# swacisko/ALGA

Measured on AMD Instinct MI355X. Metric: overlap_edges_per_sec, higher is better.
Workload: dtype u32; 1 GPU; cfg4_50M_150bp: 50000000 x 150 bp reads, genome 250000000, seed 11, err 0.00 -> 90621096 nodes (both strands, duplicates removed), min_overlap 82, rsoemo 116; generated on the device (alga_amd.workload.device_build) in 1.0 s; nodes=90621096, edges=92350115

## Files before the change

alga_amd/csrc/engine.hip:

```cpp
#include <hip/hip_runtime.h>

#include <algorithm>
#include <chrono>
#include <cstdio>
#include <cstdlib>
#include <cstring>
#include <new>
#include <string>
#include <thread>
#include <vector>

#include "engine_internal.h"
#include "prefsuf_shard.h"

using namespace alga;

namespace {

using Prepared = AlgaPrepared;

int prepare(alga_engine *e, const alga_nodes *nodes, const alga_prefsuf_params *p, hipStream_t s, Prepared &out) {
    if (!nodes || !p) return alga_fail(e, ALGA_ERR_INVALID_ARGUMENT, "nodes/params must not be NULL");
    if (nodes->n < 0) return alga_fail(e, ALGA_ERR_INVALID_ARGUMENT, "negative node count");
    if (nodes->n > 0 && (!nodes->words || !nodes->len)) return alga_fail(e, ALGA_ERR_INVALID_ARGUMENT, "words/len must not be NULL");
// ... 203 lines not shown
                HIP_TRY(e, hipEventRecord(e->ev[EV_DIR], s));
            }
            HIP_TRY(e, launch_cluster_gather(nd, cc, pp.cluster_eq, (const uint32_t *) e->cl_keys[1].p, (const uint32_t *) e->cl_vals[1].p, (const uint32_t *) e->cl_meta.p,
                                             pp.uniform_len, e->cl_store.p, (pile && e->opt_pile_skip_gather) ? (const unsigned long long *) e->cl_pile_cnt.p : nullptr, s));
            HIP_TRY(e, hipEventRecord(e->ev[EV_GATHER], s));
            if (pile) {
                if (e->pile_epoch >= 511u) {
                    HIP_TRY(e, hipMemsetAsync(e->cl_pile_tab.p, 0, e->cl_pile_tab.cap, s));
                    e->pile_epoch = 0;
                }
                e->pile_epoch++;
                const bool from_consensus = e->opt_pile_runs != 0;
                launch_pile_build(nd, cfg, cc, pp.uniform_len, (const uint32_t *) e->cl_keys[1].p, (const uint32_t *) e->cl_vals[1].p, e->cl_dir.p, e->cl_pile_rec.p, e->cl_pile_rec2.p, e->cl_pile_tab.p,
                                  e->pile_epoch, e->cl_pile_succ.p, e->cl_runs.p, pp.uniform_len - cfg.Lmin + 1, (const unsigned long long *) e->cl_pile_cnt.p,
                                  from_consensus ? (uint32_t *) e->cl_pile_own.p : nullptr, (from_consensus && e->opt_pile_runs_list) ? e->cl_pile_list.p : nullptr, s,
                                  e->opt_pile_dir >= 1, cnt + CNT_TOTAL + 1, e->pile_tab_index);
                if ((rc = alga_check_launch(e, "k_pile_build"))) return rc;
                if (keys_only) {
                    launch_pile_own_ids((const uint32_t *) e->cl_pile_own.p, (const uint32_t *) e->cl_vals[1].p, (uint64_t) nd.n, (int32_t *) e->cl_defer.p, (uint32_t) nd.n,
                                        (unsigned long long *) e->cl_pile_cnt.p, s);
                    launch_cluster_runs_list(nd, cfg, cc, (const int32_t *) e->cl_defer.p, (const unsigned long long *) e->cl_pile_cnt.p + 3, (uint32_t) nd.n, (uint32_t) e->n_cu * 16u,
                                             e->cl_runs.p, (uint8_t *) e->cl_nruns.p, s);
                    launch_cluster_keys(nd, cfg, cc, 0, nd.n, (uint32_t *) e->cl_keys[0].p, (uint32_t *) e->cl_vals[0].p, (uint32_t *) e->cl_meta.p, e->cl_runs.p,
                                        (uint8_t *) e->cl_nruns.p, s, true, (const unsigned long long *) e->cl_pile_cnt.p);
                    if ((rc = alga_check_launch(e, "k_node_runs (own lists)"))) return rc;
                }
                if (e->opt_pile_check && from_consensus)
                    launch_pile_check(e->cl_pile_succ.p, (uint64_t) nd.n, cc.n_buckets, e->cl_pile_tab.p, e->cl_pile_rec2.p, e->pile_epoch, e->cl_runs.p, nd.n, pp.uniform_len - cfg.Lmin + 1,
                                      (unsigned long long *) e->cl_pile_cnt.p, s);
                e->pile_n = nd.n; e->pile_words = (const void *) nd.words;
                e->pile_keys_only = keys_only; e->pile_kept_pure = false;
// ... 32 lines not shown
                if ((rc = alga_ensure(e, e->cl_defer, (size_t) (n_src + 64) * sizeof(int32_t)))) return rc;
                const uint32_t slot_stride = e->opt_stream_slots >= 4 ? (uint32_t) (n_src + 1) : 0u;
                if ((rc = alga_ensure(e, e->loc_second, (size_t) (slot_stride ? LOCAL_SLOTS_MAX - 1 : 1) * (n_src + 1) * sizeof(unsigned long long)))) return rc;
                e->loc_second_used = true;
                e->loc_slot_stride = slot_stride;
                const bool by_key = e->opt_cluster_order != 0 && src_begin == 0 && src_end == nd.n;
                const bool piled = pile && e->pile_n == nd.n && e->pile_words == (const void *) nd.words;
                if (piled) {
                    if (!all_sources) {
                        if ((rc = alga_ensure(e, e->cl_pile_side_r, (size_t) (n_src + 64) * 16))) return rc;
                        if ((rc = alga_ensure(e, e->cl_pile_cursor, 64))) return rc;
                    }
                    launch_pile_probe(nd, cfg, cc, pp.uniform_len, e->cl_pile_tab.p, e->pile_epoch, e->cl_pile_rec.p, e->cl_pile_rec2.p, e->cl_pile_succ.p,
                                      e->cl_runs.p, cnt, (uint32_t *) e->outdeg.p, (unsigned long long *) e->loc_first.p, (unsigned long long *) e->loc_second.p,
                                      (int32_t *) e->cl_defer.p, (uint32_t) n_src, (const unsigned long long *) e->cl_pile_cnt.p, e->n_cu, s, src_begin, src_end,
                                      e->cl_pile_side_r.p, (unsigned long long *) e->cl_pile_cursor.p, e->opt_pile_probe_lean != 0);
                    if ((rc = alga_check_launch(e, "k_pile_probe"))) return rc;
                    if (keys_only)
                        launch_cluster_runs_list(nd, cfg, cc, (const int32_t *) e->cl_defer.p, cnt + CNT_DEFERRED, (uint32_t) std::min<uint64_t>(n_src + 64, 0xFFFFFFFFull),
                                                 (uint32_t) e->n_cu * 16u, e->cl_runs.p, (uint8_t *) e->cl_nruns.p, s);
                }
                launch_probe_stream(nd, cfg, cc, pp.cluster_eq, e->cl_store.p, e->cl_dir.p, e->cl_runs.p, (const uint8_t *) e->cl_nruns.p,
                                    src_begin, src_end, by_key, cnt, e->n_cu, (uint32_t *) e->outdeg.p, (unsigned long long *) e->loc_first.p,
                                    (unsigned long long *) e->loc_second.p, (int32_t *) e->cl_defer.p, (uint32_t) n_src,
                                    piled ? (const unsigned long long *) e->cl_pile_cnt.p : nullptr, s, slot_stride);
                if ((rc = alga_check_launch(e, "k_probe_stream"))) return rc;
                if (piled) {
                    if ((rc = alga_ensure(e, e->cl_defer2, (size_t) (n_src + 64) * sizeof(int32_t)))) return rc;
                    pure_streamed = launch_probe_stream_list(nd, cfg, cc, pp.cluster_eq, e->cl_store.p, e->cl_dir.p, e->cl_runs.p, (const uint8_t *) e->cl_nruns.p, (int32_t *) e->cl_defer.p,
                                             (uint32_t) n_src, cnt, e->n_cu, (uint32_t *) e->outdeg.p, (unsigned long long *) e->loc_first.p,
                                             (unsigned long long *) e->loc_second.p, (int32_t *) e->cl_defer2.p, (const unsigned long long *) e->cl_pile_cnt.p, s, slot_stride, src_begin,
// ... 325 lines not shown
    } else if (!strcmp(name, "pile")) {
        e->opt_pile = (value == 2 || value == 3) ? (int) value : (value != 0);
    } else if (!strcmp(name, "pile_runs")) {
        e->opt_pile_runs = value != 0;
    } else if (!strcmp(name, "pile_runs_list")) {
        e->opt_pile_runs_list = value != 0;
    } else if (!strcmp(name, "pile_dir")) {
        if (value < 0 || value > 2) return alga_fail(e, ALGA_ERR_INVALID_ARGUMENT, "option pile_dir: 0 directory records, 1 k_pile_build from the keys, 2 ... and no directory for a pure pile build");
        e->opt_pile_dir = (int) value;
    } else if (!strcmp(name, "pile_deg_fold")) {
        e->opt_pile_deg_fold = value != 0;
    } else if (!strcmp(name, "emit_fused")) {
        e->opt_emit_fused = value != 0;
    } else if (!strcmp(name, "pile_probe_lean")) {
        e->opt_pile_probe_lean = value != 0;
    } else if (!strcmp(name, "pile_stream_by_id")) {
        e->opt_pile_stream_by_id = value != 0;
    } else if (!strcmp(name, "pile_check")) {
        e->opt_pile_check = value != 0;
    } else if (!strcmp(name, "pile_skip_gather")) {
        e->opt_pile_skip_gather = value != 0;
    } else if (!strcmp(name, "cluster_order")) {
        e->opt_cluster_order = value != 0;
    } else if (!strcmp(name, "local_big_max")) {
        e->big_limit = value < 0 ? -1 : (int) std::min<int64_t>(value, 1 << 20);
    } else if (!strcmp(name, "shard_bucket_max")) {
        e->opt_shard_dmax = (int) std::max<int64_t>(1, std::min<int64_t>(value, 4096));
    } else if (!strcmp(name, "rsort_variant")) {
        if (value < 0 || value > 1) return alga_fail(e, ALGA_ERR_INVALID_ARGUMENT, "option rsort_variant: 0 tiles of 8192 pairs, 1 tiles of 16384 pairs");
        rsort_set_variant((int) value);
// ... 737 lines not shown
```

alga_amd/csrc/engine_internal.h:

```cpp
#pragma once
#include <hip/hip_runtime.h>

#include <cstdio>
#include <algorithm>
#include <string>
#include <vector>
#include <unordered_map>

#include "../../include/alga_amd.h"
#include "prefsuf_common.h"
#include "prefsuf_kernels.h"
#include "pkb_kernels.h"

struct DevBuf {
    void  *p = nullptr;
    size_t cap = 0;
};

enum { EV_START = 0, EV_SEED, EV_PROBE, EV_GROUP, EV_REDUCE, EV_EMIT, EV_PAIRS, EV_KEYS, EV_SORT, EV_GATHER, EV_DIR, EV_SAMPLE, EV_COUNT };
constexpr int ALGA_STAGE_THREADS = 8;

struct alga_engine {
    std::vector<DevBuf *> owned;
    int         device = -1;
// ... 26 lines not shown
    bool   store_timed = false;
    bool   pile_keys_only = false, pile_kept_pure = false;
    int    opt_pile_range = 1;
    int    opt_pile_skip_gather = 1;
    int    opt_pile = 1;
    int    opt_pile_runs = 1;
    int    opt_pile_runs_list = 1;
    DevBuf cl_pile_list;
    int    opt_pile_deg_fold = 1;
    int    opt_emit_fused = 1;
    int    opt_pile_dir = 2;
    bool   dir_late = false;
    bool   pile_tab_index = false;
    int    opt_pile_stream_by_id = 0;
    int    opt_pile_probe_lean = 1;
    bool   pile_deg_pending = false;
    int    opt_pile_check = 0;
    bool   expect_pairwise = false;
    DevBuf cl_pile_side_r, cl_pile_cursor;
    DevBuf cl_pile_own;
    int    opt_pkb_legacy = 0;
    int    opt_own_sort = 1;
    int    opt_test_presort_oom = 0;
    int    opt_test_pile_oom = 0;
    bool   pile_timed = false;
    DevBuf cl_pile_succ;
    DevBuf cl_pile_rec2;
    DevBuf cl_pile_rec, cl_pile_cnt, cl_pile_tab;
    uint32_t pile_epoch = 0;
    int32_t pile_n = -1; const void *pile_words = nullptr;
// ... 228 lines not shown
```

alga_amd/csrc/prefsuf_kernels.h:

```cpp
#pragma once
#include <hip/hip_runtime.h>
#include <stddef.h>
#include <stdint.h>
#include "prefsuf_common.h"

namespace alga {

struct alga_edge_dev { int32_t src, dst, offset; };

void launch_restride(const uint32_t *in, int stride_in, uint32_t *out, int stride_out, uint64_t n, hipStream_t s);
void launch_widen_len(const void *in, int elem_bytes , int32_t *out, uint64_t n, hipStream_t s);
void launch_compact_edges(const alga_edge_dev *edges, int32_t n, uint64_t n_edges, uint8_t *deg, uint32_t *dst, uint8_t *off, unsigned long long *bad, hipStream_t s);
void launch_expand_twins(const uint32_t *in, int stride_in, const int32_t *len , uint32_t *out, int stride_out, uint64_t n_pairs, hipStream_t s);
void launch_node_stats(const NodesDev &nd, unsigned long long *counters, int *max_len , hipStream_t s);

uint32_t seed_buckets_for(uint64_t live_nodes, int fill_x10);
uint32_t seed_filter_bits_for(uint64_t live_nodes);
void launch_seed_build(const NodesDev &nd, const PrefSufCfg &cfg, unsigned long long *table, uint32_t n_buckets, uint32_t *filter,
                       uint32_t filter_bits, hipStream_t s);

struct ProbeBig { int32_t *list; uint32_t list_cap; uint32_t count; void *items; uint32_t item_cap; };
int    local_item_capacity();
int    local_big_limit();
size_t probe_big_bytes(int n_cu, uint32_t count, int local, uint32_t item_cap);
// ... 43 lines not shown
void       launch_pile_deg(int32_t n, unsigned long long *first, uint32_t *deg, const unsigned long long *pile_cnt, hipStream_t s);
bool       pile_plan(const PrefSufCfg &cfg, const ClusterCfg &cc, int eq, int uniform_len, bool masks);
size_t     pile_record_bytes(uint64_t n);
size_t     pile_table_bytes(uint32_t n_buckets);
void       launch_pile_sample(const NodesDev &nd, const ClusterCfg &cc, int uniform_len, const uint32_t *skeys , const uint32_t *sids , const void *dir,
                              unsigned long long *pile_cnt , int no_sample, hipStream_t s,
                              bool from_keys = false );
constexpr int PILE_CNT_WORDS = 6;
size_t     pile_own_mask_bytes(uint64_t n);
size_t     pile_list_bytes(uint64_t n);
void       launch_pile_build(const NodesDev &nd, const PrefSufCfg &cfg, const ClusterCfg &cc, int uniform_len, const uint32_t *skeys, const uint32_t *sids, const void *dir, void *rec,
                             void *rec2 , void *tab, uint32_t epoch, void *side, const void *runs, int nwin, const unsigned long long *pile_cnt,
                             uint32_t *own_mask ,
                             void *plist , hipStream_t s,
                             bool from_keys = false , unsigned long long *bad_flag = nullptr,
                             bool full_record = false );
void       launch_pile_own_ids(const uint32_t *own_mask, const uint32_t *sids, uint64_t n_entries, int32_t *list, uint32_t cap, unsigned long long *pile_cnt, hipStream_t s);
void       launch_pile_check(const void *side, uint64_t n_entries, uint32_t n_buckets, const void *tab, const void *rec2, uint32_t epoch, const void *runs, int n_nodes, int nwin,
                             unsigned long long *pile_cnt, hipStream_t s);
bool       launch_probe_stream_list(const NodesDev &nd, const PrefSufCfg &cfg, const ClusterCfg &cc, int eq, const void *store, const void *dir, const void *runs, const uint8_t *nruns,
                                    int32_t *src_list, uint32_t list_cap, unsigned long long *counters, int n_cu, uint32_t *deg, unsigned long long *first,
                                    unsigned long long *second, int32_t *defer2, const unsigned long long *pile_cnt, hipStream_t s, uint32_t slot_stride = 0,
                                    int32_t src_base = 0 ,
                                    const uint32_t *skeys = nullptr, const uint32_t *sids = nullptr, int uniform_len = 0, bool by_id = false,
                                    const void *tab = nullptr , uint32_t epoch = 0);
void       launch_pile_probe(const NodesDev &nd, const PrefSufCfg &cfg, const ClusterCfg &cc, int uniform_len, const void *tab, uint32_t epoch, const void *rec, const void *rec2, const void *side,
                             const void *runs, unsigned long long *counters, uint32_t *deg, unsigned long long *first, unsigned long long *second, int32_t *defer_list,
                             uint32_t defer_cap, const unsigned long long *pile_cnt, int n_cu, hipStream_t s, int32_t src_begin, int32_t src_end,
                             void *side_range , unsigned long long *cursor ,
                             bool lean = true );

size_t     rsort_u32_pairs_temp_bytes(uint64_t n);
void       rsort_set_variant(int v);
hipError_t rsort_u32_pairs(void *temp, size_t temp_bytes, const uint32_t *keys_in, uint32_t *keys_out, const uint32_t *vals_in, uint32_t *vals_out, uint64_t n,
                           int begin_bit, hipStream_t s);
size_t     sort_u32_pairs_temp_bytes(uint64_t n);
hipError_t sort_u32_pairs(void *temp, size_t temp_bytes, const uint32_t *keys_in, uint32_t *keys_out, const uint32_t *vals_in, uint32_t *vals_out,
                          uint64_t n, int begin_bit , hipStream_t s, bool own_sort = true );
size_t     rsort_u64_pairs_temp_bytes(uint64_t n);
hipError_t rsort_u64_pairs(void *temp, size_t temp_bytes, const unsigned long long *keys_in, unsigned long long *keys_out, const unsigned long long *vals_in,
                           unsigned long long *vals_out, uint64_t n, int bits, hipStream_t s);
hipError_t rsort_u32_u64(void *temp, size_t temp_bytes, const uint32_t *keys_in, uint32_t *keys_out, const unsigned long long *vals_in, unsigned long long *vals_out,
                         uint64_t n, int begin_bit, int end_bit, hipStream_t s);
size_t     sort_u64_pairs_temp_bytes(uint64_t n, int bits);
hipError_t sort_u64_pairs(void *temp, size_t temp_bytes, const unsigned long long *keys_in, unsigned long long *keys_out,
// ... 42 lines not shown
```

alga_amd/csrc/prefsuf_pile.hip:

```cpp
#include <hip/hip_runtime.h>
#include <algorithm>
#include "prefsuf_common.h"
#include "prefsuf_kernels.h"
#include "prefsuf_device.h"
#include "prefsuf_cluster_device.h"

namespace alga {

constexpr int PB_TILE = 192, PB_HALO = 64, PB_THREADS = PB_TILE + PB_HALO;
constexpr int PILE_SW = 13;
constexpr int PILE_MAXSUB = 4;
constexpr int PILE_EQ = 3;

__device__ __forceinline__ bool pile_declines(const unsigned long long *pile_cnt) { return pile_cnt_declines(pile_cnt); }

__device__ __forceinline__ uint32_t pile_who(uint32_t group, uint32_t w, uint32_t n_buckets, uint64_t n_entries) {
    return group == 0u ? min(w, n_buckets) : (uint32_t) min((uint64_t) w, n_entries) | 0x80000000u;
}

__device__ __forceinline__ void load_row9(const NodesDev &nd, uint32_t id, uint32_t (&row)[9]) {
    const uint32_t *rp = nd.words + (size_t) id * nd.stride;
    if ((nd.stride & 3) == 0 && nd.stride >= 12 && ((uintptr_t) nd.words & 15u) == 0) {
        const uint4 v0 = reinterpret_cast<const uint4 *>(rp)[0], v1 = reinterpret_cast<const uint4 *>(rp)[1];
        row[0] = v0.x; row[1] = v0.y; row[2] = v0.z; row[3] = v0.w; row[4] = v1.x; row[5] = v1.y; row[6] = v1.z; row[7] = v1.w;
// ... 328 lines not shown
                    last_key = k1[r]; last_pos = kpos; c1_last = c1;
                    n++;
                }
            }
        }
    }
    ok = ok && n >= 1 && n <= PILE_RUNS;
    pile_list_store(line, l4.x, ok, n, ok_, kc_, c1_last);
}

constexpr int PR_TILE = 3072;
constexpr int PR_TKW = 21;
constexpr int PR_RCAP = 14;
constexpr int PR_SEGS = 32;

template <int RS, int RW>
__device__ __forceinline__ void pile_consensus_one(uint32_t who, bool in, uint32_t *row, uint32_t (*stk)[TK_ROWS], uint16_t (*rbuf)[TK_ROWS], int t, const uint4 *__restrict__ side,
                                                   uint64_t n_entries, uint4 *__restrict__ tab, const uint4 *__restrict__ rec, uint4 *__restrict__ rec2, const ClusterCfg &cc, int U,
                                                   int Lmin, uint32_t *__restrict__ own_mask) {
    const int fs = cc.idx_shift - CL_MBITS;
    const int step = max(16, min(64, cc.w) & ~15);
    const bool further = (who >> 31) != 0u;
    const uint32_t slot = who & 0x7FFFFFFFu;
    uint4 *line = tab + (size_t) (further ? 0u : who) * 8;
    const uint4 *src = further ? rec + (size_t) slot * 4 : (const uint4 *) line;
    uint32_t S[PILE_SW + 1];
    unsigned long long rm = 0ull;
    {
        const uint4 l0 = src[0], l1 = src[1], l2 = src[2], l3 = src[3];
        S[0] = l0.x; S[1] = l0.y; S[2] = l0.z; S[3] = l0.w; S[4] = l1.x; S[5] = l1.y; S[6] = l1.z; S[7] = l1.w;
        S[8] = l2.x; S[9] = l2.y; S[10] = l2.z; S[11] = l2.w; S[12] = l3.x; S[13] = 0u;
        rm = !in ? 0ull : (further ? (((unsigned long long) l3.w << 32) | l3.z) : (((unsigned long long) l3.z << 32) | l3.y));
    }
    const bool act = in && rm != 0ull;
    const int m_min = act ? __clzll((long long) rm) : 0, m_max = act ? 63 - __builtin_ctzll(rm) : 0;
    const int len_v = U + m_max - m_min;
    const int nwin = len_v - Lmin + 1;
    {
        const int ob = 2 * (64 - m_max), w0 = ob >> 5, sh = ob & 31;
        uint32_t m1 = 0u - (uint32_t) (w0 & 1), m2 = 0u - (uint32_t) ((w0 >> 1) & 1), m4 = 0u - (uint32_t) ((w0 >> 2) & 1);
        asm volatile("" : "+v"(m1), "+v"(m2), "+v"(m4));
        uint32_t y1[PILE_SW + 1], y2[PILE_SW + 1], y[PILE_SW + 1];
#pragma unroll
        for (int k = 0; k <= PILE_SW; k++) y1[k] = ((k + 1 <= PILE_SW ? S[k + 1] : 0u) & m1) | (S[k] & ~m1);
// ... 31 lines not shown
        }
    }
    ok = ok && n >= 1 && n <= PILE_RUNS;
    if (in && further) {
        uint4 *l2 = rec2 + (size_t) slot * 4 - 4;
        pile_list_store(l2, 0u, ok, n, key_, kc_, (uint32_t) (nwin - m_max + 64));
        if (!ok) {
            const uint64_t jb = slot >= 3u ? (uint64_t) slot - 3u : 0ull;
            for (uint64_t j2 = jb; j2 < jb + 64u + 3u && j2 < n_entries; j2++) {
                const uint4 s2 = side[j2];
                if ((s2.z >> 31) && ((s2.z >> 16) & 3u) != 0u && s2.w == slot) atomicOr(&own_mask[j2 >> 5], 1u << (j2 & 31u));
            }
        }
    } else if (in) {
        uint32_t *lw = reinterpret_cast<uint32_t *>(line);
        pile_list_store(line, lw[16], ok, n, key_, kc_, (uint32_t) (nwin - m_max + 64));
        if (!ok) {
            lw[16] = lw[16] & 255u;
            const uint32_t cntb = min(lw[16] & 255u, 64u), e0b = lw[17];
            for (uint32_t i2 = 0; i2 < cntb; i2++) {
                const uint64_t j2 = (uint64_t) e0b + i2;
                if (j2 < n_entries) { const uint4 s2 = side[j2]; if ((s2.z >> 31) && ((s2.z >> 16) & 3u) == 0u) atomicOr(&own_mask[j2 >> 5], 1u << (j2 & 31u)); }
            }
        }
    }
}

__global__ void __launch_bounds__(TK_ROWS) k_pile_runs_consensus(const uint4 *__restrict__ side, uint64_t n_entries, uint32_t n_buckets, uint4 *__restrict__ tab, const uint4 *__restrict__ rec,
                                                                 uint4 *__restrict__ rec2, ClusterCfg cc, int U, int Lmin,
                                                                 const unsigned long long *__restrict__ pile_cnt, uint32_t *__restrict__ own_mask) {
    if (pile_declines(pile_cnt)) return;
    __shared__ uint32_t s[TK_ROWS][PR_TKW];
    __shared__ uint32_t stk[2 * (NR_STACK + 1)][TK_ROWS];
    __shared__ uint16_t rbuf[PR_RCAP + 1][TK_ROWS];
// ... 3 lines not shown
    if (t == 0) sN = 0u;
    __syncthreads();
    const uint64_t base = (uint64_t) blockIdx.x * PR_TILE;
#pragma unroll
    for (int q = 0; q < PR_TILE / TK_ROWS; q++) {
        const uint64_t j = base + (uint64_t) q * TK_ROWS + (uint64_t) t;
        if (j < n_entries) {
            const uint4 sd = side[j];
            if ((sd.z >> 30) & 1u) sList[atomicAdd(&sN, 1u)] = pile_who((sd.z >> 16) & 3u, sd.w, n_buckets, n_entries);
        }
    }
    __syncthreads();
    const int np = (int) sN;
    for (int c0 = 0; c0 < np; c0 += TK_ROWS) {
        const bool in = c0 + t < np;
        pile_consensus_one<1, 0>(sList[in ? c0 + t : 0], in, s[t], stk, rbuf, t, side, n_entries, tab, rec, rec2, cc, U, Lmin, own_mask);
    }
}

__global__ void __launch_bounds__(TK_ROWS) k_pile_runs_consensus_list(const uint32_t *__restrict__ plist, const uint32_t *__restrict__ pcount, uint32_t n_segs, const uint4 *__restrict__ side,
                                                                      uint64_t n_entries, uint4 *__restrict__ tab, const uint4 *__restrict__ rec, uint4 *__restrict__ rec2, ClusterCfg cc,
                                                                      int U, int Lmin, const unsigned long long *__restrict__ pile_cnt, uint32_t *__restrict__ own_mask) {
    if (pile_declines(pile_cnt)) return;
    __shared__ uint32_t s[PILE_SW][TK_ROWS];
    __shared__ uint32_t stk[2 * (NR_STACK + 1)][TK_ROWS];
    __shared__ uint16_t rbuf[PR_RCAP + 1][TK_ROWS];
    __shared__ uint32_t sOff[PR_SEGS + 1];
    const int t = (int) threadIdx.x;
    const uint32_t seg0 = blockIdx.x * PR_SEGS;
    if (t < 64) {
        const uint32_t g = seg0 + (uint32_t) t;
        uint32_t c = (t < PR_SEGS && g < n_segs) ? min(pcount[g], (uint32_t) PB_THREADS) : 0u;
#pragma unroll
        for (int d = 1; d < PR_SEGS; d <<= 1) { const uint32_t o = __shfl_up(c, d); if (t >= d) c += o; }
        if (t < PR_SEGS) sOff[t + 1] = c;
        if (t == 0) sOff[0] = 0u;
    }
    __syncthreads();
    const int np = (int) sOff[PR_SEGS];
    for (int c0 = 0; c0 < np; c0 += TK_ROWS) {
        const int i = c0 + t;
        const bool in = i < np;
        int g = 0;
#pragma unroll
        for (int b = PR_SEGS / 2; b >= 1; b >>= 1) g += (g + b <= PR_SEGS - 1 && (int) sOff[g + b] <= i) ? b : 0;
        const uint32_t who = in ? plist[(size_t) (seg0 + (uint32_t) g) * PB_THREADS + (uint32_t) (i - (int) sOff[g])] : 0u;
        pile_consensus_one<TK_ROWS, PILE_SW>(who, in, &s[0][t], stk, rbuf, t, side, n_entries, tab, rec, rec2, cc, U, Lmin, own_mask);
    }
}

__global__ void __launch_bounds__(256) k_pile_own_ids(const uint32_t *__restrict__ own_mask, const uint32_t *__restrict__ sids, uint64_t n_entries, int32_t *__restrict__ out, uint32_t cap,
                                                      unsigned long long *__restrict__ count, const unsigned long long *__restrict__ pile_cnt) {
    if (pile_declines(pile_cnt)) return;
    __shared__ uint32_t sTot, sBase;
    const uint64_t words = (n_entries + 31) / 32;
    const uint64_t w0 = (uint64_t) blockIdx.x * 1024 + threadIdx.x;
    uint32_t mw[4];
    uint32_t mine = 0u;
#pragma unroll
    for (int q = 0; q < 4; q++) { const uint64_t w = w0 + (uint64_t) q * 256; mw[q] = w < words ? own_mask[w] : 0u; mine += (uint32_t) __popc(mw[q]); }
    if (threadIdx.x == 0) sTot = 0u;
    __syncthreads();
// ... 67 lines not shown
}

#ifndef PP_WAVES_N
#define PP_WAVES_N 4
#endif
constexpr int PP_WAVES = PP_WAVES_N;
constexpr int PP_LSTRIDE = 20;
#ifndef PP_OCC
#define PP_OCC 4
#endif
#ifdef PP_NO_COMPACT
constexpr bool PP_HOME_ANY_SLOT = true;
#else
constexpr bool PP_HOME_ANY_SLOT = false;
#endif
template <bool LEAN>
__global__ void __launch_bounds__(PP_WAVES * 64, PP_OCC) k_pile_probe(PrefSufCfg cfg, ClusterCfg cc, int U, NodesDev nd, uint64_t n_entries, uint64_t n_mine, int n_nodes,
                                                                 const uint4 *__restrict__ tab, uint32_t epoch, const uint4 *__restrict__ rec, const uint4 *__restrict__ rec2,
                                                                 const uint4 *__restrict__ side, const uint4 *__restrict__ side_src, const uint2 *__restrict__ runs, ProbeOut o,
                                                                 int32_t *__restrict__ defer_list, uint32_t defer_cap, const unsigned long long *__restrict__ pile_cnt) {
    __shared__ __attribute__((aligned(16))) uint32_t sL[PP_WAVES][4 + 64 * PP_LSTRIDE + 12];
    __shared__ uint32_t sBk[PP_WAVES][64];
    __shared__ int32_t sDefer[PP_WAVES][128];
    if (blockIdx.x == 0 && threadIdx.x == 0) { o.counters[CNT_PILE_BUCKETS] = pile_cnt[0]; o.counters[CNT_PILE_IRREGULAR] = pile_cnt[1]; o.counters[CNT_PILE_OWN] = pile_cnt[3]; }
    if (pile_declines(pile_cnt)) return;
    const int wave = (int) (threadIdx.x >> 6), lane = lane_id();
    uint32_t *sl = sL[wave] + 4;
    for (int k = lane; k < 4 + 64 * PP_LSTRIDE + 12; k += 64) sL[wave][k] = 0u;
    wave_lds_fence();
    uint64_t st_rec = 0;
    int n_defer = 0;
// ... 226 lines not shown
        const uint4 R3 = *reinterpret_cast<const uint4 *>(sl + li * PP_LSTRIDE + 12);
        const uint32_t y = R3.w, tag = rk[a] & 31u;
        const bool live = ((vmask >> a) & 1u) != 0u && (y >> 23) == epoch;
        dfr = dfr || (live && ((y >> 22) & 1u) != 0u);
        const uint32_t ns = ((y >> 20) & 3u) + 1u;
        uint32_t mt = ((y & 31u) == tag ? 1u : 0u) | ((ns >= 2u && ((y >> 5) & 31u) == tag) ? 2u : 0u) | ((ns >= 3u && ((y >> 10) & 31u) == tag) ? 4u : 0u) |
                      ((ns >= 4u && ((y >> 15) & 31u) == tag) ? 8u : 0u);
        mt = (live && !dfr) ? mt : 0u;
        more |= (mt & ~1u) << (4 * a);
        const bool on = (mt & 1u) != 0u;
        if (__ballot(on) == 0ull) continue;
        const bool home = (!LEAN || PP_HOME_ANY_SLOT || a == 0) && on && row_from_pile && !got_row && ((ry[a] >> 8) & 255u) == 0u;
        got_row = got_row || home;
        take_record(li * PP_LSTRIDE, ((unsigned long long) R3.z << 32) | R3.y, a, 0u, ry[a], on, home);
    }
    {
        const uint4 *rp = run_list_of(next_side);
#pragma unroll
        for (int c = 0; c < CL_RMAX / 2; c++) Qr[c] = rp[c];
    }
    dfr = dfr || (active && !got_row);
    more = dfr ? 0u : more;
    while (__ballot(more != 0u) != 0ull) {
        const bool on = more != 0u;
        const int bit = on ? __builtin_ctz(more) : 0;
        more &= more - 1u;
        const int a = bit >> 2;
        const uint32_t g = (uint32_t) (bit & 3);
        uint32_t ya = ry[0], ka = rk[0];
#pragma unroll
        for (int k = 1; k < CL_RMAX; k++) { ya = a == k ? ry[k] : ya; ka = a == k ? rk[k] : ka; }
        const uint32_t xa = reinterpret_cast<const uint32_t *>(tab)[(size_t) min(ka >> cc.idx_shift, cc.n_buckets) * 32 + 17];
        const uint64_t se = min((uint64_t) xa + g, last);
        const uint4 Q0 = rec[se * 4], Q1 = rec[se * 4 + 1], Q2 = rec[se * 4 + 2], Q3 = rec[se * 4 + 3];
        uint4 *mine = reinterpret_cast<uint4 *>(sl + lane * PP_LSTRIDE);
        mine[0] = Q0; mine[1] = Q1; mine[2] = Q2; mine[3] = Q3;
        wave_lds_fence();
        take_record(lane * PP_LSTRIDE, ((unsigned long long) Q3.w << 32) | Q3.z, a, g, ya, on, false);
        wave_lds_fence();
    }
    const unsigned long long kept = occ & ~smear_up(occ, G);
    const int nkept = __popcll(kept);
    if (nkept > 2) dfr = true;
    auto lookup = [&](int d) -> uint32_t {
        uint32_t ya = 0u, ka = 0u, ga = 0u;
#pragma unroll
        for (int k = 0; k < CL_RMAX; k++) {
            const bool in = ((vmask >> k) & 1u) != 0u && d >= (int) ((ry[k] >> 8) & 255u) && d < (int) ((ry[k] >> 16) & 255u);
            ya = in ? ry[k] : ya; ka = in ? rk[k] : ka; ga = in ? (grp >> (2 * k)) & 3u : ga;
        }
        const uint4 dd = tab[(size_t) min(ka >> cc.idx_shift, cc.n_buckets) * 8 + 4];
        const int mm = (int) (ya & 255u) - d;
        const int cl = (mm >> 3) & 7;
        const uint32_t b0 = ((cl < 4 ? dd.z : dd.w) >> (8 * (cl & 3))) & 255u;
        const uint32_t b1 = cl >= 7 ? (dd.x & 127u) : ((((cl + 1) < 4 ? dd.z : dd.w) >> (8 * ((cl + 1) & 3))) & 255u);
        uint32_t id = 0xFFFFFFFFu;
        for (uint32_t e = b0; e < b1 && e < 64u; e++) {
            const uint64_t ei = min((uint64_t) dd.y + e, last);
            const uint4 sd = side[ei];
            if ((int) ((sd.z >> 8) & 63u) == mm && ((sd.z >> 16) & 3u) == ga) id = sd.x;
        }
        return id;
    };
    unsigned long long slot_val = LOCAL_FIRST_NONE;
    if (active && !dfr && nkept > 0) {
        const int d1 = __builtin_ctzll(kept);
        int p1_home = 0;
#pragma unroll
        for (int k = 0; k < CL_RMAX; k++) p1_home = (((vmask >> k) & 1u) != 0u && ((ry[k] >> 8) & 255u) == 0u) ? (int) ((ry[k] >> 16) & 255u) : p1_home;
        const bool by_succ = d1 < p1_home && (int) (my.z & 255u) == d1 && my.y != 0xFFFFFFFFu;
#ifdef PP_LK
        const int d2 = nkept == 2 ? 63 - __clzll((long long) kept) : -1;
        const int dA = by_succ ? d2 : d1, dB = by_succ ? -1 : d2;
        uint32_t idA = 0xFFFFFFFFu, idB = 0xFFFFFFFFu;
        if (dA >= 0) idA = lookup(dA);
        if (dB >= 0) idB = lookup(dB);
        const uint32_t id1 = by_succ ? my.y : idA;
        const uint32_t id2 = by_succ ? idA : idB;
        bool two = false;
        if (nkept == 2) {
#else
        const uint32_t id1 = by_succ ? my.y : lookup(d1);
        uint32_t id2 = 0u;
        int d2 = 0;
        bool two = false;
        if (nkept == 2) {
            d2 = 63 - __clzll((long long) kept);
            id2 = lookup(d2);
#endif
            const int ds0 = U - cfg.rsoemo + 1;
            const unsigned long long lowm = ds0 <= 0 ? 0ull : (ds0 >= 64 ? ~0ull : ((1ull << ds0) - 1ull));
            two = d2 < ds0 || __popcll(occ & ((1ull << d2) - 1ull) & ~lowm) < 3;
        }
        if (id1 == 0xFFFFFFFFu || (nkept == 2 && id2 == 0xFFFFFFFFu)) dfr = true;
        else {
            slot_val = ((unsigned long long) id1 << 32) | (uint32_t) d1 | (two ? 0x100u : 0u);
            if (two) o.second[Bs - o.src_base] = ((unsigned long long) id2 << 32) | (uint32_t) d2;
            st_rec += two ? 2 : 1;
        }
    }
    if (have) o.first[Bs - o.src_base] = slot_val;
    dfr = dfr && nr_code != 0;
    const uint64_t dm = __ballot(dfr);
    if (dm != 0ull) {
// ... 38 lines not shown
void launch_pile_sample(const NodesDev &nd, const ClusterCfg &cc, int uniform_len, const uint32_t *skeys, const uint32_t *sids, const void *dir, unsigned long long *pile_cnt,
                        int no_sample, hipStream_t s, bool from_keys) {
    (void) hipMemsetAsync(pile_cnt, 0, PILE_CNT_WORDS * sizeof(unsigned long long), s);
    const uint64_t n_entries = nd.n > 0 ? (uint64_t) nd.n : 0;
    if (no_sample == 2) hipLaunchKernelGGL(k_pile_sample_force, dim3(1), dim3(1), 0, s, pile_cnt, 100ull, 1ull);
    if (n_entries == 0 || no_sample) return;
    const uint64_t tiles = (n_entries + PB_TILE - 1) / PB_TILE;
    const dim3 sample((unsigned) std::max<uint64_t>(1, std::min<uint64_t>(tiles, std::max<uint64_t>(64, tiles / 32)))), block(PB_THREADS);
    hipLaunchKernelGGL((from_keys ? k_pile_build<true, true> : k_pile_build<true, false>), sample, block, 0, s, nd, skeys, sids, n_entries, (const uint4 *) dir, cc, uniform_len, (uint4 *) nullptr,
                       (uint4 *) nullptr, 0u, (uint4 *) nullptr, pile_cnt, (uint32_t *) nullptr, (uint32_t *) nullptr, (uint32_t *) nullptr, (unsigned long long *) nullptr, 0u);
    hipLaunchKernelGGL(k_pile_sample_close, dim3(1), dim3(1), 0, s, pile_cnt);
}

void launch_pile_build(const NodesDev &nd, const PrefSufCfg &cfg, const ClusterCfg &cc, int uniform_len, const uint32_t *skeys, const uint32_t *sids, const void *dir, void *rec, void *rec2,
                       void *tab, uint32_t epoch, void *side, const void *runs, int nwin, const unsigned long long *pile_cnt, uint32_t *own_mask, void *plist, hipStream_t s,
                       bool from_keys, unsigned long long *bad_flag, bool full_record) {
    const uint64_t n_entries = nd.n > 0 ? (uint64_t) nd.n : 0;
    if (n_entries == 0) return;
    const uint64_t tiles = (n_entries + PB_TILE - 1) / PB_TILE;
    if (!own_mask) plist = nullptr;
    uint32_t *pl = (uint32_t *) plist, *pc = pl ? pl + tiles * PB_THREADS : nullptr;
    if (own_mask) (void) hipMemsetAsync(own_mask, 0, pile_own_mask_bytes(n_entries), s);
    hipLaunchKernelGGL((from_keys ? k_pile_build<false, true> : k_pile_build<false, false>), dim3((unsigned) tiles), dim3(PB_THREADS), 0, s, nd, skeys, sids, n_entries, (const uint4 *) dir, cc, uniform_len,
                       (uint4 *) rec, (uint4 *) tab, epoch, (uint4 *) side, const_cast<unsigned long long *>(pile_cnt), own_mask, pl, pc, bad_flag, full_record ? 1u : 0u);
    if (pl)
        hipLaunchKernelGGL(k_pile_runs_consensus_list, dim3((unsigned) ((tiles + PR_SEGS - 1) / PR_SEGS)), dim3(TK_ROWS), 0, s, (const uint32_t *) pl, (const uint32_t *) pc, (uint32_t) tiles,
                           (const uint4 *) side, n_entries, (uint4 *) tab, (const uint4 *) rec, (uint4 *) rec2, cc, uniform_len, cfg.Lmin, pile_cnt, own_mask);
    else if (own_mask)
        hipLaunchKernelGGL(k_pile_runs_consensus, dim3((unsigned) ((n_entries + PR_TILE - 1) / PR_TILE)), dim3(TK_ROWS), 0, s, (const uint4 *) side, n_entries, cc.n_buckets, (uint4 *) tab,
                           (const uint4 *) rec, (uint4 *) rec2, cc, uniform_len, cfg.Lmin, pile_cnt, own_mask);
    else
        hipLaunchKernelGGL(k_pile_runs, dim3((unsigned) ((n_entries + 255) / 256)), dim3(256), 0, s, (const uint4 *) side, n_entries, cc.n_buckets, (uint4 *) tab, (const uint2 *) runs, nd.n, nwin, pile_cnt);
}

size_t pile_own_mask_bytes(uint64_t n) { return (size_t) ((n + 31) / 32 + 1024) * 4; }

size_t pile_list_bytes(uint64_t n) { const uint64_t tiles = (n + PB_TILE - 1) / PB_TILE; return (size_t) (tiles * (PB_THREADS + 1) + 64) * 4; }

void launch_pile_own_ids(const uint32_t *own_mask, const uint32_t *sids, uint64_t n_entries, int32_t *list, uint32_t cap, unsigned long long *pile_cnt, hipStream_t s) {
    if (n_entries == 0) return;
    const uint64_t words = (n_entries + 31) / 32;
    hipLaunchKernelGGL(k_pile_own_ids, dim3((unsigned) ((words + 1023) / 1024)), dim3(256), 0, s, own_mask, sids, n_entries, list, cap, pile_cnt + 3, (const unsigned long long *) pile_cnt);
// ... 35 lines not shown
    }
    __syncthreads();
    uint32_t run = 0;
#pragma unroll
    for (int k = 0; k < PSR_IPT; k++) {
        uint32_t mine = run;
        for (int w = 0; w < 4; w++) { if (w < wave) mine += cnt[k * 4 + w]; run += cnt[k * 4 + w]; }
        const unsigned long long at = base + mine + before[k];
        if (in[k] && at < out_cap) out[at] = v[k];
    }
}

void launch_pile_probe(const NodesDev &nd, const PrefSufCfg &cfg, const ClusterCfg &cc, int uniform_len, const void *tab, uint32_t epoch, const void *rec, const void *rec2,
                       const void *side, const void *runs, unsigned long long *counters, uint32_t *deg, unsigned long long *first, unsigned long long *second,
                       int32_t *defer_list, uint32_t defer_cap, const unsigned long long *pile_cnt, int n_cu, hipStream_t s, int32_t src_begin, int32_t src_end,
                       void *side_range, unsigned long long *cursor, bool lean) {
    const uint64_t n_entries = nd.n > 0 ? (uint64_t) nd.n : 0;
    if (n_entries == 0 || src_end <= src_begin) return;
    ProbeOut o{};
    o.counters = counters; o.deg = deg; o.first = first; o.second = second; o.src_base = src_begin;
    uint64_t n_mine = n_entries;
    const void *side_src = side;
    if (src_begin != 0 || src_end != nd.n) {
        n_mine = (uint64_t) (src_end - src_begin);
        (void) hipMemsetAsync(cursor, 0, sizeof(unsigned long long), s);
        hipLaunchKernelGGL(k_pile_side_range, dim3((unsigned) ((n_entries + 256 * PSR_IPT - 1) / (256 * PSR_IPT))), dim3(256), 0, s, (const uint4 *) side, n_entries,
                           (uint32_t) src_begin, (uint32_t) src_end, (uint4 *) side_range, n_mine, cursor, pile_cnt);
        side_src = side_range;
    }
    const uint64_t tiles = (n_mine + PP_WAVES * 64 - 1) / (PP_WAVES * 64);
    const dim3 grid((unsigned) std::max<uint64_t>(1, std::min<uint64_t>(tiles, (uint64_t) std::max(1, n_cu) * (PP_OCC * 4 / PP_WAVES)))), block(PP_WAVES * 64);
    hipLaunchKernelGGL(lean ? k_pile_probe<true> : k_pile_probe<false>, grid, block, 0, s, cfg, cc, uniform_len, nd, n_entries, n_mine, nd.n, (const uint4 *) tab, epoch, (const uint4 *) rec, (const uint4 *) rec2,
                       (const uint4 *) side, (const uint4 *) side_src, (const uint2 *) runs, o, defer_list, defer_cap, pile_cnt);
}

void launch_pile_deg(int32_t n, unsigned long long *first, uint32_t *deg, const unsigned long long *pile_cnt, hipStream_t s) {
    if (n <= 0) return;
    hipLaunchKernelGGL(k_pile_deg, dim3((unsigned) (((int64_t) n + 255) / 256)), dim3(256), 0, s, n, first, deg, pile_cnt);
}

}
```

Measured before the change: 5.279 billion edges/s.

## Prefetch pile probe table loads and batch tail lookups; add runs-ahead consensus option

The pile probe kernel gains a TAIL variant, enabled by default. It loads the next bucket's first-entry index one iteration ahead, and it resolves the final one or two successor-id lookups with batched, unrolled side-table reads pinned in registers instead of serial lookup calls. Separately, the consensus builder is split into load and compute phases, with an optional software-pipelined loop (off by default) that prefetches the next chunk's record. The aim is to hide global-memory latency on dependent loads, at the cost of more registers, possible occupancy loss, and extra speculative loads.

```diff
diff --git a/alga_amd/csrc/engine.hip b/alga_amd/csrc/engine.hip
--- a/alga_amd/csrc/engine.hip
+++ b/alga_amd/csrc/engine.hip
@@ -241,7 +241,7 @@
                 launch_pile_build(nd, cfg, cc, pp.uniform_len, (const uint32_t *) e->cl_keys[1].p, (const uint32_t *) e->cl_vals[1].p, e->cl_dir.p, e->cl_pile_rec.p, e->cl_pile_rec2.p, e->cl_pile_tab.p,
                                   e->pile_epoch, e->cl_pile_succ.p, e->cl_runs.p, pp.uniform_len - cfg.Lmin + 1, (const unsigned long long *) e->cl_pile_cnt.p,
                                   from_consensus ? (uint32_t *) e->cl_pile_own.p : nullptr, (from_consensus && e->opt_pile_runs_list) ? e->cl_pile_list.p : nullptr, s,
-                                  e->opt_pile_dir >= 1, cnt + CNT_TOTAL + 1, e->pile_tab_index);
+                                  e->opt_pile_dir >= 1, cnt + CNT_TOTAL + 1, e->pile_tab_index, e->opt_pile_runs_ahead != 0);
                 if ((rc = alga_check_launch(e, "k_pile_build"))) return rc;
                 if (keys_only) {
                     launch_pile_own_ids((const uint32_t *) e->cl_pile_own.p, (const uint32_t *) e->cl_vals[1].p, (uint64_t) nd.n, (int32_t *) e->cl_defer.p, (uint32_t) nd.n,
@@ -304,7 +304,7 @@
                     launch_pile_probe(nd, cfg, cc, pp.uniform_len, e->cl_pile_tab.p, e->pile_epoch, e->cl_pile_rec.p, e->cl_pile_rec2.p, e->cl_pile_succ.p,
                                       e->cl_runs.p, cnt, (uint32_t *) e->outdeg.p, (unsigned long long *) e->loc_first.p, (unsigned long long *) e->loc_second.p,
                                       (int32_t *) e->cl_defer.p, (uint32_t) n_src, (const unsigned long long *) e->cl_pile_cnt.p, e->n_cu, s, src_begin, src_end,
-                                      e->cl_pile_side_r.p, (unsigned long long *) e->cl_pile_cursor.p, e->opt_pile_probe_lean != 0);
+                                      e->cl_pile_side_r.p, (unsigned long long *) e->cl_pile_cursor.p, e->opt_pile_probe_lean != 0, e->opt_pile_probe_tail != 0);
                     if ((rc = alga_check_launch(e, "k_pile_probe"))) return rc;
                     if (keys_only)
                         launch_cluster_runs_list(nd, cfg, cc, (const int32_t *) e->cl_defer.p, cnt + CNT_DEFERRED, (uint32_t) std::min<uint64_t>(n_src + 64, 0xFFFFFFFFull),
@@ -660,6 +660,10 @@
         e->opt_emit_fused = value != 0;
     } else if (!strcmp(name, "pile_probe_lean")) {
         e->opt_pile_probe_lean = value != 0;
+    } else if (!strcmp(name, "pile_probe_tail")) {
+        e->opt_pile_probe_tail = value != 0;
+    } else if (!strcmp(name, "pile_runs_ahead")) {
+        e->opt_pile_runs_ahead = value != 0;
     } else if (!strcmp(name, "pile_stream_by_id")) {
         e->opt_pile_stream_by_id = value != 0;
     } else if (!strcmp(name, "pile_check")) {
diff --git a/alga_amd/csrc/engine_internal.h b/alga_amd/csrc/engine_internal.h
--- a/alga_amd/csrc/engine_internal.h
+++ b/alga_amd/csrc/engine_internal.h
@@ -64,6 +64,8 @@
     bool   pile_tab_index = false;
     int    opt_pile_stream_by_id = 0;
     int    opt_pile_probe_lean = 1;
+    int    opt_pile_probe_tail = 1;
+    int    opt_pile_runs_ahead = 0;
     bool   pile_deg_pending = false;
     int    opt_pile_check = 0;
     bool   expect_pairwise = false;
diff --git a/alga_amd/csrc/prefsuf_kernels.h b/alga_amd/csrc/prefsuf_kernels.h
--- a/alga_amd/csrc/prefsuf_kernels.h
+++ b/alga_amd/csrc/prefsuf_kernels.h
@@ -81,7 +81,8 @@
                              uint32_t *own_mask ,
                              void *plist , hipStream_t s,
                              bool from_keys = false , unsigned long long *bad_flag = nullptr,
-                             bool full_record = false );
+                             bool full_record = false ,
+                             bool runs_ahead = false );
 void       launch_pile_own_ids(const uint32_t *own_mask, const uint32_t *sids, uint64_t n_entries, int32_t *list, uint32_t cap, unsigned long long *pile_cnt, hipStream_t s);
 void       launch_pile_check(const void *side, uint64_t n_entries, uint32_t n_buckets, const void *tab, const void *rec2, uint32_t epoch, const void *runs, int n_nodes, int nwin,
                              unsigned long long *pile_cnt, hipStream_t s);
@@ -95,7 +96,7 @@
                              const void *runs, unsigned long long *counters, uint32_t *deg, unsigned long long *first, unsigned long long *second, int32_t *defer_list,
                              uint32_t defer_cap, const unsigned long long *pile_cnt, int n_cu, hipStream_t s, int32_t src_begin, int32_t src_end,
                              void *side_range , unsigned long long *cursor ,
-                             bool lean = true );
+                             bool lean = true , bool tail = false );
 
 size_t     rsort_u32_pairs_temp_bytes(uint64_t n);
 void       rsort_set_variant(int v);
diff --git a/alga_amd/csrc/prefsuf_pile.hip b/alga_amd/csrc/prefsuf_pile.hip
--- a/alga_amd/csrc/prefsuf_pile.hip
+++ b/alga_amd/csrc/prefsuf_pile.hip
@@ -366,20 +366,25 @@
 constexpr int PR_RCAP = 14;
 constexpr int PR_SEGS = 32;
 
+__device__ __forceinline__ void pile_consensus_load(uint32_t who, const uint4 *__restrict__ tab, const uint4 *__restrict__ rec, uint4 &l0, uint4 &l1, uint4 &l2, uint4 &l3, uint32_t &w16) {
+    const bool further = (who >> 31) != 0u;
+    const uint4 *src = further ? rec + (size_t) (who & 0x7FFFFFFFu) * 4 : tab + (size_t) who * 8;
+    l0 = src[0]; l1 = src[1]; l2 = src[2]; l3 = src[3];
+    w16 = reinterpret_cast<const uint32_t *>(src)[further ? 0 : 16];
+}
+
 template <int RS, int RW>
-__device__ __forceinline__ void pile_consensus_one(uint32_t who, bool in, uint32_t *row, uint32_t (*stk)[TK_ROWS], uint16_t (*rbuf)[TK_ROWS], int t, const uint4 *__restrict__ side,
-                                                   uint64_t n_entries, uint4 *__restrict__ tab, const uint4 *__restrict__ rec, uint4 *__restrict__ rec2, const ClusterCfg &cc, int U,
-                                                   int Lmin, uint32_t *__restrict__ own_mask) {
+__device__ __forceinline__ void pile_consensus_make(uint32_t who, bool in, const uint4 l0, const uint4 l1, const uint4 l2, const uint4 l3, const uint32_t w16, uint32_t *row, uint32_t (*stk)[TK_ROWS], uint16_t (*rbuf)[TK_ROWS], int t,
+                                                    const uint4 *__restrict__ side, uint64_t n_entries, uint4 *__restrict__ tab, uint4 *__restrict__ rec2, const ClusterCfg &cc, int U,
+                                                    int Lmin, uint32_t *__restrict__ own_mask) {
     const int fs = cc.idx_shift - CL_MBITS;
     const int step = max(16, min(64, cc.w) & ~15);
     const bool further = (who >> 31) != 0u;
     const uint32_t slot = who & 0x7FFFFFFFu;
     uint4 *line = tab + (size_t) (further ? 0u : who) * 8;
-    const uint4 *src = further ? rec + (size_t) slot * 4 : (const uint4 *) line;
     uint32_t S[PILE_SW + 1];
     unsigned long long rm = 0ull;
     {
-        const uint4 l0 = src[0], l1 = src[1], l2 = src[2], l3 = src[3];
         S[0] = l0.x; S[1] = l0.y; S[2] = l0.z; S[3] = l0.w; S[4] = l1.x; S[5] = l1.y; S[6] = l1.z; S[7] = l1.w;
         S[8] = l2.x; S[9] = l2.y; S[10] = l2.z; S[11] = l2.w; S[12] = l3.x; S[13] = 0u;
         rm = !in ? 0ull : (further ? (((unsigned long long) l3.w << 32) | l3.z) : (((unsigned long long) l3.z << 32) | l3.y));
@@ -441,10 +446,11 @@
         }
     } else if (in) {
         uint32_t *lw = reinterpret_cast<uint32_t *>(line);
-        pile_list_store(line, lw[16], ok, n, key_, kc_, (uint32_t) (nwin - m_max + 64));
+        uint32_t entries = w16;
+        asm volatile("" : "+v"(entries));
+        pile_list_store(line, entries, ok, n, key_, kc_, (uint32_t) (nwin - m_max + 64));
         if (!ok) {
-            lw[16] = lw[16] & 255u;
-            const uint32_t cntb = min(lw[16] & 255u, 64u), e0b = lw[17];
+            const uint32_t cntb = min(entries & 255u, 64u), e0b = lw[17];
             for (uint32_t i2 = 0; i2 < cntb; i2++) {
                 const uint64_t j2 = (uint64_t) e0b + i2;
                 if (j2 < n_entries) { const uint4 s2 = side[j2]; if ((s2.z >> 31) && ((s2.z >> 16) & 3u) == 0u) atomicOr(&own_mask[j2 >> 5], 1u << (j2 & 31u)); }
@@ -478,13 +484,18 @@
     const int np = (int) sN;
     for (int c0 = 0; c0 < np; c0 += TK_ROWS) {
         const bool in = c0 + t < np;
-        pile_consensus_one<1, 0>(sList[in ? c0 + t : 0], in, s[t], stk, rbuf, t, side, n_entries, tab, rec, rec2, cc, U, Lmin, own_mask);
+        const uint32_t who = sList[in ? c0 + t : 0];
+        uint4 l0, l1, l2, l3;
+        uint32_t w16;
+        pile_consensus_load(who, tab, rec, l0, l1, l2, l3, w16);
+        pile_consensus_make<1, 0>(who, in, l0, l1, l2, l3, w16, s[t], stk, rbuf, t, side, n_entries, tab, rec2, cc, U, Lmin, own_mask);
     }
 }
 
 __global__ void __launch_bounds__(TK_ROWS) k_pile_runs_consensus_list(const uint32_t *__restrict__ plist, const uint32_t *__restrict__ pcount, uint32_t n_segs, const uint4 *__restrict__ side,
                                                                       uint64_t n_entries, uint4 *__restrict__ tab, const uint4 *__restrict__ rec, uint4 *__restrict__ rec2, ClusterCfg cc,
-                                                                      int U, int Lmin, const unsigned long long *__restrict__ pile_cnt, uint32_t *__restrict__ own_mask) {
+                                                                      int U, int Lmin, const unsigned long long *__restrict__ pile_cnt, uint32_t *__restrict__ own_mask,
+                                                                      int ahead ) {
     if (pile_declines(pile_cnt)) return;
     __shared__ uint32_t s[PILE_SW][TK_ROWS];
     __shared__ uint32_t stk[2 * (NR_STACK + 1)][TK_ROWS];
@@ -502,14 +513,36 @@
     }
     __syncthreads();
     const int np = (int) sOff[PR_SEGS];
+    auto who_of = [&](int c0) -> uint32_t {
+        const int i = c0 + t;
+        int g = 0;
+#pragma unroll
+        for (int b = PR_SEGS / 2; b >= 1; b >>= 1) g += (g + b <= PR_SEGS - 1 && (int) sOff[g + b] <= i) ? b : 0;
+        return i < np ? plist[(size_t) (seg0 + (uint32_t) g) * PB_THREADS + (uint32_t) (i - (int) sOff[g])] : 0u;
+    };
+    if (!ahead) {
+        for (int c0 = 0; c0 < np; c0 += TK_ROWS) {
+            const uint32_t who = who_of(c0);
+            uint4 l0, l1, l2, l3;
+            uint32_t w16;
+            pile_consensus_load(who, tab, rec, l0, l1, l2, l3, w16);
+            pile_consensus_make<TK_ROWS, PILE_SW>(who, c0 + t < np, l0, l1, l2, l3, w16, &s[0][t], stk, rbuf, t, side, n_entries, tab, rec2, cc, U, Lmin, own_mask);
+        }
+        return;
+    }
+    if (np <= 0) return;
+    uint32_t who1 = who_of(0), who2 = who_of(TK_ROWS);
+    uint4 n0, n1, n2, n3;
+    uint32_t nw;
+    pile_consensus_load(who1, tab, rec, n0, n1, n2, n3, nw);
     for (int c0 = 0; c0 < np; c0 += TK_ROWS) {
-        const int i = c0 + t;
-        const bool in = i < np;
-        int g = 0;
-#pragma unroll
-        for (int b = PR_SEGS / 2; b >= 1; b >>= 1) g += (g + b <= PR_SEGS - 1 && (int) sOff[g + b] <= i) ? b : 0;
-        const uint32_t who = in ? plist[(size_t) (seg0 + (uint32_t) g) * PB_THREADS + (uint32_t) (i - (int) sOff[g])] : 0u;
-        pile_consensus_one<TK_ROWS, PILE_SW>(who, in, &s[0][t], stk, rbuf, t, side, n_entries, tab, rec, rec2, cc, U, Lmin, own_mask);
+        const uint32_t who = who1;
+        const uint4 l0 = n0, l1 = n1, l2 = n2, l3 = n3;
+        const uint32_t w16 = nw;
+        who1 = who2;
+        if (c0 + TK_ROWS < np) pile_consensus_load(who1, tab, rec, n0, n1, n2, n3, nw);
+        if (c0 + 2 * TK_ROWS < np) who2 = who_of(c0 + 2 * TK_ROWS);
+        pile_consensus_make<TK_ROWS, PILE_SW>(who, c0 + t < np, l0, l1, l2, l3, w16, &s[0][t], stk, rbuf, t, side, n_entries, tab, rec2, cc, U, Lmin, own_mask);
     }
 }
 
@@ -607,7 +640,8 @@
 #else
 constexpr bool PP_HOME_ANY_SLOT = false;
 #endif
-template <bool LEAN>
+constexpr int PP_TAIL_K = 4;
+template <bool LEAN, bool TAIL>
 __global__ void __launch_bounds__(PP_WAVES * 64, PP_OCC) k_pile_probe(PrefSufCfg cfg, ClusterCfg cc, int U, NodesDev nd, uint64_t n_entries, uint64_t n_mine, int n_nodes,
                                                                  const uint4 *__restrict__ tab, uint32_t epoch, const uint4 *__restrict__ rec, const uint4 *__restrict__ rec2,
                                                                  const uint4 *__restrict__ side, const uint4 *__restrict__ side_src, const uint2 *__restrict__ runs, ProbeOut o,
@@ -864,13 +898,22 @@
         got_row = got_row || home;
         take_record(li * PP_LSTRIDE, ((unsigned long long) R3.z << 32) | R3.y, a, 0u, ry[a], on, home);
     }
+    dfr = dfr || (active && !got_row);
+    more = dfr ? 0u : more;
+    auto first_entry_of = [&](uint32_t m) -> uint32_t {
+        const int a = m != 0u ? __builtin_ctz(m) >> 2 : 0;
+        uint32_t ka = 0u;
+#pragma unroll
+        for (int k = 0; k < CL_RMAX; k++) ka |= rk[k] & (0u - (uint32_t) (a == k));
+        return reinterpret_cast<const uint32_t *>(tab)[(size_t) (m != 0u ? min(ka >> cc.idx_shift, cc.n_buckets) : cc.n_buckets) * 32 + 17];
+    };
+    uint32_t xa_next = 0u;
+    if constexpr (TAIL) xa_next = first_entry_of(more);
     {
         const uint4 *rp = run_list_of(next_side);
 #pragma unroll
         for (int c = 0; c < CL_RMAX / 2; c++) Qr[c] = rp[c];
     }
-    dfr = dfr || (active && !got_row);
-    more = dfr ? 0u : more;
     while (__ballot(more != 0u) != 0ull) {
         const bool on = more != 0u;
         const int bit = on ? __builtin_ctz(more) : 0;
@@ -880,9 +923,10 @@
         uint32_t ya = ry[0], ka = rk[0];
 #pragma unroll
         for (int k = 1; k < CL_RMAX; k++) { ya = a == k ? ry[k] : ya; ka = a == k ? rk[k] : ka; }
-        const uint32_t xa = reinterpret_cast<const uint32_t *>(tab)[(size_t) min(ka >> cc.idx_shift, cc.n_buckets) * 32 + 17];
+        const uint32_t xa = TAIL ? xa_next : reinterpret_cast<const uint32_t *>(tab)[(size_t) min(ka >> cc.idx_shift, cc.n_buckets) * 32 + 17];
         const uint64_t se = min((uint64_t) xa + g, last);
         const uint4 Q0 = rec[se * 4], Q1 = rec[se * 4 + 1], Q2 = rec[se * 4 + 2], Q3 = rec[se * 4 + 3];
+        if constexpr (TAIL) xa_next = first_entry_of(more);
         uint4 *mine = reinterpret_cast<uint4 *>(sl + lane * PP_LSTRIDE);
         mine[0] = Q0; mine[1] = Q1; mine[2] = Q2; mine[3] = Q3;
         wave_lds_fence();
@@ -912,6 +956,57 @@
         }
         return id;
     };
+    uint32_t lk_id1 = 0xFFFFFFFFu, lk_id2 = 0xFFFFFFFFu;
+    if constexpr (TAIL) {
+        const bool fin = active && !dfr && nkept > 0;
+        const int d1 = fin ? __builtin_ctzll(kept) : 0, d2 = (fin && nkept == 2) ? 63 - __clzll((long long) kept) : 0;
+        uint32_t y1 = 0u, k1 = 0u, g1 = 0u, y2 = 0u, k2 = 0u, g2 = 0u;
+        int p1_home = 0;
+#pragma unroll
+        for (int k = 0; k < CL_RMAX; k++) {
+            const bool v = ((vmask >> k) & 1u) != 0u;
+            const int p0 = (int) ((ry[k] >> 8) & 255u), p1 = (int) ((ry[k] >> 16) & 255u);
+            const uint32_t gk = (grp >> (2 * k)) & 3u;
+            p1_home = (v && p0 == 0) ? p1 : p1_home;
+            const bool in1 = v && d1 >= p0 && d1 < p1, in2 = v && d2 >= p0 && d2 < p1;
+            y1 = in1 ? ry[k] : y1; k1 = in1 ? rk[k] : k1; g1 = in1 ? gk : g1;
+            y2 = in2 ? ry[k] : y2; k2 = in2 ? rk[k] : k2; g2 = in2 ? gk : g2;
+        }
+        const bool need1 = fin && !(d1 < p1_home && (int) (my.z & 255u) == d1 && my.y != 0xFFFFFFFFu), need2 = fin && nkept == 2;
+        if (__ballot(need1 || need2) != 0ull) {
+            uint4 dd1 = tab[(size_t) (need1 ? min(k1 >> cc.idx_shift, cc.n_buckets) : cc.n_buckets) * 8 + 4];
+            uint4 dd2 = tab[(size_t) (need2 ? min(k2 >> cc.idx_shift, cc.n_buckets) : cc.n_buckets) * 8 + 4];
+            asm volatile("" : "+v"(dd1.x), "+v"(dd1.y), "+v"(dd1.z), "+v"(dd1.w), "+v"(dd2.x), "+v"(dd2.y), "+v"(dd2.z), "+v"(dd2.w));
+            auto class_of = [&](const uint4 &dd, int mm, bool need, uint32_t &b0, uint32_t &b1) {
+                const int cl = (mm >> 3) & 7;
+                b0 = ((cl < 4 ? dd.z : dd.w) >> (8 * (cl & 3))) & 255u;
+                b1 = cl >= 7 ? (dd.x & 127u) : ((((cl + 1) < 4 ? dd.z : dd.w) >> (8 * ((cl + 1) & 3))) & 255u);
+                b1 = need ? min(b1, 64u) : 0u;
+                b0 = need ? b0 : 0u;
+            };
+            const int mm1 = (int) (y1 & 255u) - d1, mm2 = (int) (y2 & 255u) - d2;
+            uint32_t e1, e1_end, e2, e2_end;
+            class_of(dd1, mm1, need1, e1, e1_end);
+            class_of(dd2, mm2, need2, e2, e2_end);
+            do {
+                uint32_t cx1[PP_TAIL_K], cz1[PP_TAIL_K], cx2[PP_TAIL_K], cz2[PP_TAIL_K];
+#pragma unroll
+                for (int i = 0; i < PP_TAIL_K; i++) {
+                    const uint4 *c1 = side + min((uint64_t) dd1.y + e1 + (uint32_t) i, last), *c2 = side + min((uint64_t) dd2.y + e2 + (uint32_t) i, last);
+                    cx1[i] = c1->x; cz1[i] = c1->z; cx2[i] = c2->x; cz2[i] = c2->z;
+                }
+                static_assert(PP_TAIL_K == 4, "the batch is pinned word by word");
+                asm volatile("" : "+v"(cx1[0]), "+v"(cz1[0]), "+v"(cx1[1]), "+v"(cz1[1]), "+v"(cx1[2]), "+v"(cz1[2]), "+v"(cx1[3]), "+v"(cz1[3]),
+                                  "+v"(cx2[0]), "+v"(cz2[0]), "+v"(cx2[1]), "+v"(cz2[1]), "+v"(cx2[2]), "+v"(cz2[2]), "+v"(cx2[3]), "+v"(cz2[3]));
+#pragma unroll
+                for (int i = 0; i < PP_TAIL_K; i++) {
+                    if (e1 + (uint32_t) i < e1_end && (int) ((cz1[i] >> 8) & 63u) == mm1 && ((cz1[i] >> 16) & 3u) == g1) lk_id1 = cx1[i];
+                    if (e2 + (uint32_t) i < e2_end && (int) ((cz2[i] >> 8) & 63u) == mm2 && ((cz2[i] >> 16) & 3u) == g2) lk_id2 = cx2[i];
+                }
+                e1 += PP_TAIL_K; e2 += PP_TAIL_K;
+            } while (__ballot(e1 < e1_end || e2 < e2_end) != 0ull);
+        }
+    }
     unsigned long long slot_val = LOCAL_FIRST_NONE;
     if (active && !dfr && nkept > 0) {
         const int d1 = __builtin_ctzll(kept);
@@ -919,25 +1014,13 @@
 #pragma unroll
         for (int k = 0; k < CL_RMAX; k++) p1_home = (((vmask >> k) & 1u) != 0u && ((ry[k] >> 8) & 255u) == 0u) ? (int) ((ry[k] >> 16) & 255u) : p1_home;
         const bool by_succ = d1 < p1_home && (int) (my.z & 255u) == d1 && my.y != 0xFFFFFFFFu;
-#ifdef PP_LK
-        const int d2 = nkept == 2 ? 63 - __clzll((long long) kept) : -1;
-        const int dA = by_succ ? d2 : d1, dB = by_succ ? -1 : d2;
-        uint32_t idA = 0xFFFFFFFFu, idB = 0xFFFFFFFFu;
-        if (dA >= 0) idA = lookup(dA);
-        if (dB >= 0) idB = lookup(dB);
-        const uint32_t id1 = by_succ ? my.y : idA;
-        const uint32_t id2 = by_succ ? idA : idB;
-        bool two = false;
-        if (nkept == 2) {
-#else
-        const uint32_t id1 = by_succ ? my.y : lookup(d1);
+        const uint32_t id1 = by_succ ? my.y : (TAIL ? lk_id1 : lookup(d1));
         uint32_t id2 = 0u;
         int d2 = 0;
         bool two = false;
         if (nkept == 2) {
             d2 = 63 - __clzll((long long) kept);
-            id2 = lookup(d2);
-#endif
+            id2 = TAIL ? lk_id2 : lookup(d2);
             const int ds0 = U - cfg.rsoemo + 1;
             const unsigned long long lowm = ds0 <= 0 ? 0ull : (ds0 >= 64 ? ~0ull : ((1ull << ds0) - 1ull));
             two = d2 < ds0 || __popcll(occ & ((1ull << d2) - 1ull) & ~lowm) < 3;
@@ -1006,7 +1089,7 @@
 
 void launch_pile_build(const NodesDev &nd, const PrefSufCfg &cfg, const ClusterCfg &cc, int uniform_len, const uint32_t *skeys, const uint32_t *sids, const void *dir, void *rec, void *rec2,
                        void *tab, uint32_t epoch, void *side, const void *runs, int nwin, const unsigned long long *pile_cnt, uint32_t *own_mask, void *plist, hipStream_t s,
-                       bool from_keys, unsigned long long *bad_flag, bool full_record) {
+                       bool from_keys, unsigned long long *bad_flag, bool full_record, bool runs_ahead) {
     const uint64_t n_entries = nd.n > 0 ? (uint64_t) nd.n : 0;
     if (n_entries == 0) return;
     const uint64_t tiles = (n_entries + PB_TILE - 1) / PB_TILE;
@@ -1017,7 +1100,7 @@
                        (uint4 *) rec, (uint4 *) tab, epoch, (uint4 *) side, const_cast<unsigned long long *>(pile_cnt), own_mask, pl, pc, bad_flag, full_record ? 1u : 0u);
     if (pl)
         hipLaunchKernelGGL(k_pile_runs_consensus_list, dim3((unsigned) ((tiles + PR_SEGS - 1) / PR_SEGS)), dim3(TK_ROWS), 0, s, (const uint32_t *) pl, (const uint32_t *) pc, (uint32_t) tiles,
-                           (const uint4 *) side, n_entries, (uint4 *) tab, (const uint4 *) rec, (uint4 *) rec2, cc, uniform_len, cfg.Lmin, pile_cnt, own_mask);
+                           (const uint4 *) side, n_entries, (uint4 *) tab, (const uint4 *) rec, (uint4 *) rec2, cc, uniform_len, cfg.Lmin, pile_cnt, own_mask, runs_ahead ? 1 : 0);
     else if (own_mask)
         hipLaunchKernelGGL(k_pile_runs_consensus, dim3((unsigned) ((n_entries + PR_TILE - 1) / PR_TILE)), dim3(TK_ROWS), 0, s, (const uint4 *) side, n_entries, cc.n_buckets, (uint4 *) tab,
                            (const uint4 *) rec, (uint4 *) rec2, cc, uniform_len, cfg.Lmin, pile_cnt, own_mask);
@@ -1083,7 +1166,7 @@
 void launch_pile_probe(const NodesDev &nd, const PrefSufCfg &cfg, const ClusterCfg &cc, int uniform_len, const void *tab, uint32_t epoch, const void *rec, const void *rec2,
                        const void *side, const void *runs, unsigned long long *counters, uint32_t *deg, unsigned long long *first, unsigned long long *second,
                        int32_t *defer_list, uint32_t defer_cap, const unsigned long long *pile_cnt, int n_cu, hipStream_t s, int32_t src_begin, int32_t src_end,
-                       void *side_range, unsigned long long *cursor, bool lean) {
+                       void *side_range, unsigned long long *cursor, bool lean, bool tail) {
     const uint64_t n_entries = nd.n > 0 ? (uint64_t) nd.n : 0;
     if (n_entries == 0 || src_end <= src_begin) return;
     ProbeOut o{};
@@ -1099,7 +1182,7 @@
     }
     const uint64_t tiles = (n_mine + PP_WAVES * 64 - 1) / (PP_WAVES * 64);
     const dim3 grid((unsigned) std::max<uint64_t>(1, std::min<uint64_t>(tiles, (uint64_t) std::max(1, n_cu) * (PP_OCC * 4 / PP_WAVES)))), block(PP_WAVES * 64);
-    hipLaunchKernelGGL(lean ? k_pile_probe<true> : k_pile_probe<false>, grid, block, 0, s, cfg, cc, uniform_len, nd, n_entries, n_mine, nd.n, (const uint4 *) tab, epoch, (const uint4 *) rec, (const uint4 *) rec2,
+    hipLaunchKernelGGL((lean ? (tail ? k_pile_probe<true, true> : k_pile_probe<true, false>) : k_pile_probe<false, false>), grid, block, 0, s, cfg, cc, uniform_len, nd, n_entries, n_mine, nd.n, (const uint4 *) tab, epoch, (const uint4 *) rec, (const uint4 *) rec2,
                        (const uint4 *) side, (const uint4 *) side_src, (const uint2 *) runs, o, defer_list, defer_cap, pile_cnt);
 }
 
```

Result: faster. 5.515 billion edges/s (median of 6 runs) (+4.5%).
